# FitSNAP/FitSNAP

Measured on AMD Instinct MI355X. Metric: training rows/sec through A^T A + solve, 1000000 x 128 fp64 in total over the GPUs (strong scaling), higher is better.
Workload: dtype f64

## Files before the change

fitsnap_amd/build.py:

```python
from __future__ import annotations

import hashlib
import os
import shutil
import subprocess
import sys

HERE = os.path.dirname(os.path.abspath(__file__))
CSRC = os.path.join(HERE, "csrc")
LIBDIR = os.path.join(HERE, "_lib")
LIBNAME = "libfsnap_hip.so"
SOURCES = ["fsnap_syrk_quad.hip:0", "fsnap_syrk_quad.hip:1", "fsnap_syrk_quad.hip:2", "fsnap_syrk.hip", "fsnap_syrk_short.hip", "fsnap_rows.hip", "fsnap_chol.hip", "fsnap_trsm.hip", "fsnap_fused.hip", "fsnap_merr.hip", "fsnap_cand.hip", "fsnap_uq.hip", "fsnap_loco.hip", "fsnap_path.hip", "fsnap_joint.hip", "fsnap_select.hip", "fsnap_mcmc.hip", "fsnap_capi.cpp", "fsnap_comm.cpp", "fsnap_p2p.cpp",
           "fsnap_rowspace.cpp", "fsnap_rowspace_host.cpp", "fsnap_solve.cpp"]
HEADERS = ["fsnap_kernels.h", "fsnap_device_common.h", "fsnap_rowvar_body.h", "fsnap_ctx.h", "fsnap_rowspace_host.h", "fsnap_condest.h", "fsnap_p2p.h", os.path.join("..", "..", "include", "fsnap_hip.h")]
ARCH = "gfx950"


def lib_path() -> str:
    return os.path.join(LIBDIR, LIBNAME)


def _hipcc() -> str:
    exe = shutil.which("hipcc") or "/opt/rocm/bin/hipcc"
    if not os.path.exists(exe):
        raise RuntimeError("hipcc not found: libfsnap_hip.so cannot be built")
    return exe


def _source_digest() -> str:
    h = hashlib.sha256()
    for name in sorted({s.split(":")[0] for s in SOURCES}) + HEADERS:
        with open(os.path.join(CSRC, name), "rb") as f:
            h.update(f.read())
    return h.hexdigest()


def build_library(force: bool = False, verbose: bool = False) -> str:
    os.makedirs(LIBDIR, exist_ok=True)
    out = lib_path()
    stamp = out + ".sha256"
    digest = _source_digest()
    if not force and os.path.exists(out) and os.path.exists(stamp):
        with open(stamp) as f:
            if f.read().strip() == digest:
                return out
    hipcc = _hipcc()
    objs = []
    common = [f"--offload-arch={ARCH}", "-O3", "-std=c++17", "-fPIC", "-I", os.path.join(HERE, "..", "include")]
    procs = []
    objdir = os.path.join(LIBDIR, "obj")
    os.makedirs(objdir, exist_ok=True)
    hh = hashlib.sha256()
    for name in HEADERS:
        with open(os.path.join(CSRC, name), "rb") as f:
            hh.update(f.read())
    for entry in SOURCES:
        src, _, part = entry.partition(":")
        obj = os.path.join(objdir, os.path.splitext(src)[0] + (f"_{part}" if part else "") + ".o")
        cmd = [hipcc, *common]
        if part:
            cmd += [f"-DFSNAP_QUAD_PART={part}"]
        if src in ("fsnap_capi.cpp", "fsnap_comm.cpp", "fsnap_p2p.cpp", "fsnap_rowspace.cpp"):
            cmd += ["-x", "hip"]
        if src in ("fsnap_solve.cpp", "fsnap_rowspace_host.cpp"):
            cmd = [hipcc, "-x", "c++", "-O3", "-std=c++17", "-fPIC", "-mavx2", "-mfma",
# ... 39 lines not shown
```

fitsnap_amd/csrc/fsnap_capi.cpp:

```cpp
#include <hip/hip_runtime.h>

#include <algorithm>
#include <cmath>
#include <atomic>
#include <chrono>
#include <cstdarg>
#include <cstdio>
#include <cstdlib>
#include <cstring>
#include <limits>
#include <new>
#include <queue>
#include <string>
#include <thread>
#include <vector>

#include "../../include/fsnap_hip.h"
#include "fsnap_kernels.h"

extern "C" int fsnap_solve_diag_tagged(int kind, double param, int64_t K, const double* G, const double* c, const double* diag,
                                       double* beta, int* rank, double* rcond_est, int upper, const void* owner,
                                       unsigned long long generation);
extern "C" int fsnap_solve_diag_upper(int kind, double param, int64_t K, const double* G, const double* c, const double* diag,
                                      double* beta, int* rank, double* rcond_est);
// ... 526 lines not shown
    a.nblocks = g.nblocks;
    a.split = g.split;
    a.chunks_per_wave = g.cpw;
    a.nontemporal = true;
    a.part = (double*)ctx->part.p;
    a.cpart = (double*)ctx->cpart.p;
    a.spart = (double*)ctx->spart.p;
    int ns = -1;
    const double* spart_src = a.spart;
    if (g.fused_pack) {
        a.fused_pack = true;
    } else {
        int npk = 0;
        if ((rc = ensure_wpack(ctx, &npk))) return rc;
        a.wpack = ctx->wpack_override ? ctx->wpack_override : (const double*)ctx->wpack.p;
        spart_src = (const double*)ctx->wpack_spart.p;
        ns = npk;
    }
    hipEvent_t* evs;
    if ((rc = fit_events(ctx, &evs))) return rc;
    if (evs) FSNAP_HIP(hipEventRecord(evs[0], ctx->stream), "hipEventRecord");
    if (g.quad && g.cluster > 1) {
        const size_t need = (size_t)g.nblocks * 4 * sizeof(int);
        if (ctx->quad_flow.bytes < need) {
            if (!ctx->quad_flow.ensure(need)) return ctx->fail(FSNAP_E_NOMEM, "hipMalloc(flow words) failed");
            FSNAP_HIP(hipMemsetAsync(ctx->quad_flow.p, 0, ctx->quad_flow.bytes, ctx->stream), "hipMemset(flow words)");
            ctx->quad_flow_tag = 0;
        }
        ctx->quad_flow_tag += 1u << 20;
        a.flow_words = (int*)ctx->quad_flow.p;
        const int flow = 2 | ((g.cluster == 2 ? 0 : 2) << 2);
        a.flow_tag = (int)(ctx->quad_flow_tag | (unsigned)flow);
    }
    if (g.shortk) FSNAP_HIP(fsnap::launch_syrk_short(a, ctx->stream), "launch fsnap_syrk_short");
    else if (g.quad) FSNAP_HIP(fsnap::launch_syrk_quad(a, ctx->stream), "launch fsnap_syrk_quad");
    else if (g.acc) FSNAP_HIP(fsnap::launch_syrk_acc(a, ctx->stream), "launch fsnap_syrk_acc");
    else FSNAP_HIP(fsnap::launch_syrk_wave_p(a, ctx->stream), "launch fsnap_syrk_wave_p");
    if (evs) FSNAP_HIP(hipEventRecord(evs[1], ctx->stream), "hipEventRecord");
    double* mirror = nullptr;
    if (want_mirror && !device_factor(ctx, ctx->K)) {
        const size_t need = ((size_t)FSNAP_PACKED_LEN(ctx->K) + (size_t)ctx->K) * 8;
        if (ctx->mirror_bytes < need) {
            if (ctx->mirror) (void)hipHostFree(ctx->mirror);
            ctx->mirror = nullptr;
            ctx->mirror_bytes = 0;
            if (hipHostMalloc((void**)&ctx->mirror, need, hipHostMallocCoherent | hipHostMallocMapped) == hipSuccess)
                ctx->mirror_bytes = need;
        }
        if (ctx->mirror && !ctx->mirror_ev && hipEventCreateWithFlags(&ctx->mirror_ev, hipEventDisableTiming) != hipSuccess)
            ctx->mirror_ev = nullptr;
        if (ctx->mirror && ctx->mirror_ev) mirror = ctx->mirror;
    }
    const bool upper_mirror = mirror != nullptr;
    FSNAP_HIP(fsnap::launch_reduce(a.part, a.cpart, spart_src, g.nblocks, cs_per_block, ns, a.K, d_packed, mirror, accumulate,
                                   ctx->stream, upper_mirror),
              "launch fsnap_reduce_partials");
    if (evs) FSNAP_HIP(hipEventRecord(evs[2], ctx->stream), "hipEventRecord");
    if (mirror) {
        FSNAP_HIP(hipEventRecord(ctx->mirror_ev, ctx->stream), "hipEventRecord");
        ctx->mirror_of = d_packed;
        ctx->mirror_K = ctx->K;
        ctx->mirror_upper = upper_mirror;
        ctx->mirror_gen = next_mirror_generation();
    }
    if (evs) ctx->t_syrk = true;
    return FSNAP_OK;
}

}

namespace fsnap {

int wpack_current(fsnap_ctx* ctx) {
    int rc, npk = 0;
    if ((rc = check_rows(ctx)) || (rc = check_weights(ctx))) return rc;
    return ensure_wpack(ctx, &npk);
}

int normal_eq_launch_on(fsnap_ctx* ctx, const double* Q, int64_t ldq, const double* qpack, double* d_packed) {
    const double* const save_A = ctx->dA;
    const int64_t save_lda = ctx->lda;
    ctx->dA = Q;
    ctx->lda = ldq;
    ctx->wpack_override = qpack;
    const int rc = launch_normal_eq(ctx, d_packed);
    ctx->wpack_override = nullptr;
    ctx->dA = save_A;
    ctx->lda = save_lda;
    return rc;
}

}

extern "C" {

int fsnap_version(void) { return 200; }

int fsnap_device_count(int* count) {
    if (!count) return FSNAP_E_ARG;
    int n = 0;
    hipError_t e = hipGetDeviceCount(&n);
    if (e != hipSuccess) {
        g_last_error = std::string("hipGetDeviceCount: ") + hipGetErrorString(e);
        *count = 0;
        return FSNAP_E_HIP;
    }
    *count = n;
    return FSNAP_OK;
}
// ... 2180 lines not shown
```

fitsnap_amd/csrc/fsnap_kernels.h:

```cpp
#pragma once
#include <hip/hip_runtime.h>
#include <stdint.h>

namespace fsnap {

struct SyrkArgs {
    const double* A;
    int64_t lda;
    const double* b;
    const double* w;
    const unsigned char* mask;
    int64_t m;
    int K;
    int nblocks;
    int split;
    int64_t chunks_per_wave;
    bool nontemporal;
    double* part;
    double* cpart;
    double* spart;
    const double* wpack = nullptr;
    int* flow_words = nullptr;
    int flow_tag = 0;
    bool fused_pack = false;
};

struct TiledArgs {
    const double* A;
    int64_t lda;
    const double* wpack;
    int64_t m;
    int K;
    int NSB;
    int npairs;
    int nsplit;
    int64_t chunks_per_split;
    bool nontemporal;
    double* part;
    double* cpart;
    const double* spart;
    int ns;
};

int syrk_num_blocks(int K);
int syrk_waves_per_simd(int K, int split);
hipError_t launch_syrk_wave_p(const SyrkArgs& a, hipStream_t st);
hipError_t launch_syrk_acc(const SyrkArgs& a, hipStream_t st);
hipError_t launch_syrk_quad(const SyrkArgs& a, hipStream_t st);
int64_t syrk_quad_max_cpg();
int syrk_quad_cluster(int K);
int64_t syrk_acc_max_fused_cpw();
hipError_t launch_syrk_short(const SyrkArgs& a, hipStream_t st);
bool syrk_short_takes(int K);
int syrk_short_phase_rows(int K);
int64_t syrk_wave_p_max_fused_cpw(int K, int wg_per_cu);
hipError_t launch_reduce(const double* part, const double* cpart, const double* spart, int nblocks,
                         int cs_per_block, int ns, int K, double* out, double* mirror, bool accumulate, hipStream_t st,
                         bool upper_mirror = false);
int pack_weights_num_blocks(int64_t m);
hipError_t launch_pack_weights(const double* b, const double* w, const unsigned char* mask, int64_t m, double* wpack,
                               double* spart, hipStream_t st);
hipError_t launch_syrk_tiled(const TiledArgs& a, hipStream_t st);
hipError_t launch_reduce_tiled(const TiledArgs& a, double* out, bool accumulate, hipStream_t st);
hipError_t launch_weight_rows(const double* A, int64_t lda, const double* b, const double* w,
                              const unsigned char* mask, int64_t m, int K, double* aw, int64_t ldaw, double* bw,
                              hipStream_t st);
hipError_t launch_assemble(const double* raw, int64_t raw_ld, int64_t nrows, const int64_t* src_row, const int* kind,
                           const int* frac, const double* dval, const double* truth, const double* weight,
                           const double* fractions, const double* blank2J, int ntypes, int ncoeff, int off, double* A,
                           int64_t lda, double* b, double* w, hipStream_t st);
size_t assemble_row_record_bytes();
hipError_t launch_assemble_bw(const double* raw, int64_t raw_ld, int64_t nrows, const int64_t* src_row, const int* kind,
                              const int* frac, const double* d, const double* truth, const double* weight, int icolref,
                              double* b, double* w, void* recs, hipStream_t st);
hipError_t launch_assemble_syrk(const double* raw, int64_t raw_ld, const void* recs, const double* dval, const double* fractions,
                                const double* blank2J, int ntypes, int ncoeff, int off, const TiledArgs& a, hipStream_t st);
hipError_t launch_mirror_copy(const double* src, int K, double* mirror, hipStream_t st);
hipError_t launch_tri_pack(const double* packed, int K, double* tri, hipStream_t st);
hipError_t launch_tri_unpack(const double* tri, int K, double* packed, hipStream_t st);
size_t chol_large_work_doubles(int n);
hipError_t launch_chol_large(const double* packed, const double* cvec, int n, double alpha, double* work, double* dsc, double* z,
                             double* beta, int* status, double* minpiv, double* host_out, bool clear_status, double* probe_out,
                             hipStream_t st);
constexpr int CHOL_PROBES = 31;
double chol_probe(int row, int p);
hipError_t launch_chol_resolve(const double* d_rhs, int n, double* work, const double* dsc, double* z, double* beta, int* status,
                               const double* minpiv, double* host_out, hipStream_t st);
hipError_t launch_chol_factor(const double* G, int n, double shift, double* work, double* dsc, int* status, double* minpiv,
                              int K16, double* Rout, hipStream_t st);
hipError_t launch_gram_scan(const double* G, int n, double* out, hipStream_t st);
int gemv_num_blocks(int64_t m);
hipError_t launch_gemv_rows(const double* A, int64_t lda, const double* beta, int64_t m, int K, double* preds,
                            const double* b, const double* w, const unsigned char* mask, double* sse_part,
                            double* uout, hipStream_t st, bool uplain = false);
int gemvT_num_blocks(int64_t m);
int residual_num_blocks(int64_t m, int K);
hipError_t launch_residual_rows(const double* A, int64_t lda, const double* beta, int64_t m, int K, const double* b,
                                const double* w, const unsigned char* mask, double* partial, double* sse_part, double* out,
                                hipStream_t st);
hipError_t launch_colsum(const double* partial, int nparts, int ncols, double* out, hipStream_t st);
hipError_t launch_expand_weights(const double* wtrain, const unsigned char* mask, const int* rank, int64_t m, double* w,
                                 hipStream_t st);
int error_stats_num_blocks(int64_t m);
hipError_t launch_error_stats(const double* truth, const double* pred, const double* wgt, const int* cat, int64_t m, int ncat,
                              int pass, const double* means, double* partial, hipStream_t st);
hipError_t launch_gemvT_rows(const double* A, int64_t lda, const double* u, int64_t m, int K, double* partial,
                             double* out, hipStream_t st);

constexpr int MERR_IID = 0, MERR_ABC = 1, MERR_FULL = 2;
constexpr int MERR_ONE_PASS_MAX_K = 288;
int merr_num_blocks(int64_t m, int K);
// ... 97 lines not shown
```

fitsnap_amd/csrc/fsnap_solve.cpp:

```cpp
#include <atomic>
#include <chrono>
#include <cstdio>
#include <cmath>
#include <cstdlib>
#include <cstdint>
#include <cstring>
#include <limits>
#include <thread>
#include <vector>

#include "../../include/fsnap_hip.h"
#include "fsnap_condest.h"

static thread_local double g_cond_info[4] = {0.0, 0.0, 0.0, 0.0};

extern "C" __attribute__((visibility("hidden"))) void fsnap_cond_note(double min_pivot, double lambda_min, int steps, int where) {
    g_cond_info[0] = min_pivot;
    g_cond_info[1] = lambda_min;
    g_cond_info[2] = (double)steps;
    g_cond_info[3] = (double)where;
}

extern "C" int fsnap_cond_info(double* info) {
    if (!info) return FSNAP_E_ARG;
// ... 183 lines not shown
                *(v8du*)(r3) = y30; *(v8du*)(r3 + 8) = y31; *(v8du*)(r3 + 16) = y32; *(v8du*)(r3 + 24) = y33;
            }
        }
        if (cw == 16) {
            for (; i + 4 <= i_end; i += 4) {
                double* r0 = a + (size_t)i * n + c0;
                double* r1 = r0 + n;
                double* r2 = r1 + n;
                double* r3 = r2 + n;
                v8d y00 = *(const v8du*)(r0), y01 = *(const v8du*)(r0 + 8);
                v8d y10 = *(const v8du*)(r1), y11 = *(const v8du*)(r1 + 8);
                v8d y20 = *(const v8du*)(r2), y21 = *(const v8du*)(r2 + 8);
                v8d y30 = *(const v8du*)(r3), y31 = *(const v8du*)(r3 + 8);
                const double* uk = a + (size_t)jb * n;
                for (int k = 0; k < nk; ++k, uk += n) {
                    const v8d u0 = *(const v8du*)(uk + c0), u1 = *(const v8du*)(uk + c0 + 8);
                    const double f0 = uk[i], f1 = uk[i + 1], f2 = uk[i + 2], f3 = uk[i + 3];
                    const v8d b0 = {f0, f0, f0, f0, f0, f0, f0, f0}, b1 = {f1, f1, f1, f1, f1, f1, f1, f1};
                    const v8d b2 = {f2, f2, f2, f2, f2, f2, f2, f2}, b3 = {f3, f3, f3, f3, f3, f3, f3, f3};
                    y00 -= b0 * u0; y01 -= b0 * u1;
                    y10 -= b1 * u0; y11 -= b1 * u1;
                    y20 -= b2 * u0; y21 -= b2 * u1;
                    y30 -= b3 * u0; y31 -= b3 * u1;
                }
                *(v8du*)(r0) = y00; *(v8du*)(r0 + 8) = y01;
                *(v8du*)(r1) = y10; *(v8du*)(r1 + 8) = y11;
                *(v8du*)(r2) = y20; *(v8du*)(r2 + 8) = y21;
                *(v8du*)(r3) = y30; *(v8du*)(r3 + 8) = y31;
            }
        }
        for (; i < i_end; ++i) {
            double* ri = a + (size_t)i * n + c0;
            const double* uk = a + (size_t)jb * n;
            for (int k = 0; k < nk; ++k, uk += n) axpy_neg(ri, uk + c0, uk[i], cw);
        }
    }
}

int chol_upper_rb(double* a, int n, double* min_piv2, int NBK) {
    double mp = std::numeric_limits<double>::infinity();
    for (int jb = 0; jb < n; jb += NBK) {
        const int je = (jb + NBK < n) ? jb + NBK : n;
        const int fail = chol_panel(a, n, jb, je, &mp);
        if (fail >= 0) {
            if (min_piv2) *min_piv2 = mp;
            return fail;
        }
        if (je < n) chol_trailing_chunks(a, n, jb, je, 0, 1);
    }
    if (min_piv2) *min_piv2 = mp;
    return -1;
}

FSNAP_CLONES void chol_solve_inv(const double* u, int n, double* x, double* inv) {
    for (int k = 0; k < n; ++k) inv[k] = 1.0 / u[(size_t)k * n + k];
    for (int k = 0; k < n; ++k) {
        const double* r = u + (size_t)k * n;
        x[k] *= inv[k];
        axpy_neg(x + k + 1, r + k + 1, x[k], n - 1 - k);
    }
    for (int i = n - 1; i >= 0; --i) {
        const double* r = u + (size_t)i * n;
        x[i] = (x[i] - dotv(r + i + 1, x + i + 1, n - 1 - i)) * inv[i];
    }
}
void chol_solve(const double* u, int n, double* x) {
    static thread_local vec inv;
    inv.resize(n);
    chol_solve_inv(u, n, x, inv.data());
}

bool lu_solve(double* a, int n, double* b) {
    std::vector<int> piv(n);
    for (int j = 0; j < n; ++j) {
        int p = j;
        double mx = std::fabs(a[(size_t)j * n + j]);
        for (int i = j + 1; i < n; ++i) {
            double v = std::fabs(a[(size_t)i * n + j]);
            if (v > mx) {
                mx = v;
                p = i;
            }
        }
        if (!(mx > 0.0) || !std::isfinite(mx)) return false;
        if (p != j) {
            for (int k = 0; k < n; ++k) std::swap(a[(size_t)j * n + k], a[(size_t)p * n + k]);
            std::swap(b[j], b[p]);
        }
        const double inv = 1.0 / a[(size_t)j * n + j];
        for (int i = j + 1; i < n; ++i) {
            double f = a[(size_t)i * n + j] * inv;
            if (f == 0.0) continue;
            a[(size_t)i * n + j] = f;
            for (int k = j + 1; k < n; ++k) a[(size_t)i * n + k] -= f * a[(size_t)j * n + k];
            b[i] -= f * b[j];
        }
    }
    for (int i = n - 1; i >= 0; --i) {
        double s = b[i];
        for (int k = i + 1; k < n; ++k) s -= a[(size_t)i * n + k] * b[k];
        b[i] = s / a[(size_t)i * n + i];
    }
    return true;
}

void jacobi_eigh(double* a, int n, double* eval, double* v) {
    for (int i = 0; i < n; ++i)
        for (int j = 0; j < n; ++j) v[(size_t)i * n + j] = (i == j) ? 1.0 : 0.0;
    for (int sweep = 0; sweep < 60; ++sweep) {
        double off = 0.0, diag = 0.0;
        for (int i = 0; i < n; ++i) {
            diag += a[(size_t)i * n + i] * a[(size_t)i * n + i];
            for (int j = i + 1; j < n; ++j) off += a[(size_t)i * n + j] * a[(size_t)i * n + j];
        }
        if (off == 0.0 || off <= 1e-34 * diag) break;
        for (int p = 0; p < n - 1; ++p) {
            for (int q = p + 1; q < n; ++q) {
                const double apq = a[(size_t)p * n + q];
                if (apq == 0.0) continue;
                const double app = a[(size_t)p * n + p], aqq = a[(size_t)q * n + q];
                if (std::fabs(apq) <= 1e-18 * std::sqrt(std::fabs(app) * std::fabs(aqq))) {
                    a[(size_t)p * n + q] = a[(size_t)q * n + p] = 0.0;
// ... 172 lines not shown

int chol_upper_rb_mt(double* a, int n, double* min_piv2, int NBK, int nt) {
    struct Shared {
        std::atomic<int> arrived{0};
        std::atomic<int> phase{0};
        std::atomic<int> fail{-1};
        double mp = std::numeric_limits<double>::infinity();
    } sh;
    auto barrier = [&](int& local_phase) {
        ++local_phase;
        if (sh.arrived.fetch_add(1, std::memory_order_acq_rel) + 1 == nt) {
            sh.arrived.store(0, std::memory_order_relaxed);
            sh.phase.store(local_phase, std::memory_order_release);
        } else {
            int spins = 0;
            while (sh.phase.load(std::memory_order_acquire) != local_phase) {
#if defined(__x86_64__)
                __builtin_ia32_pause();
#endif
                if (++spins > 4096) {
                    std::this_thread::yield();
                    spins = 0;
                }
            }
        }
    };
    auto body = [&](int t) {
        int ph = 0;
        for (int jb = 0; jb < n; jb += NBK) {
            const int je = (jb + NBK < n) ? jb + NBK : n;
            if (t == 0) {
                const int f = chol_panel_diag(a, n, jb, je, &sh.mp);
                if (f >= 0) sh.fail.store(f, std::memory_order_relaxed);
            }
            barrier(ph);
            if (sh.fail.load(std::memory_order_relaxed) >= 0) return;
            if (je < n) {
                chol_panel_tails(a, n, jb, je, t, nt);
                barrier(ph);
                chol_trailing_chunks(a, n, jb, je, t, nt);
            }
            barrier(ph);
        }
    };
    std::vector<std::thread> th;
    th.reserve(nt - 1);
    for (int t = 1; t < nt; ++t) th.emplace_back(body, t);
    body(0);
    for (auto& x : th) x.join();
    if (min_piv2) *min_piv2 = sh.mp;
    return sh.fail.load();
}

int fast_chol(double* u, int n, double* mp2) {
    static const int forced = [] {
        const char* e = std::getenv("FSNAP_CHOL_VARIANT");
        return e ? std::atoi(e) : 0;
    }();
    static const int nbk_env = [] {
        const char* e = std::getenv("FSNAP_CHOL_NBK");
        return e ? std::atoi(e) : 0;
    }();
    if (forced == 1) return chol_upper(u, n, mp2);
    if (forced == 2) return chol_upper_blocked(u, n, mp2, 64);
    if (forced == 3 || n >= 48) {
        const int nbk = nbk_env > 0 ? nbk_env : (n <= 256 ? 8 : 32);
        static const int nt_env = [] {
            const char* e = std::getenv("FSNAP_CHOL_THREADS");
            return e ? std::atoi(e) : 0;
        }();
        static const int nt_auto = [] {
            auto quota = [](const char* path, bool v2) -> bool {
                FILE* f = std::fopen(path, "r");
                if (!f) return false;
                char buf[64] = {0};
                const bool got = std::fgets(buf, sizeof buf, f) != nullptr;
                std::fclose(f);
                if (!got) return false;
                return v2 ? std::strncmp(buf, "max", 3) != 0 : std::atol(buf) > 0;
            };
            if (quota("/sys/fs/cgroup/cpu.max", true) || quota("/sys/fs/cgroup/cpu/cpu.cfs_quota_us", false)) return 1;
            const unsigned hc = std::thread::hardware_concurrency();
            return (int)(hc >= 8 ? 8 : (hc > 0 ? hc : 1));
        }();
        int nt = nt_env > 0 ? nt_env : nt_auto;
        if (nt > n / 160) nt = n / 160;
        if (nt > 1) return chol_upper_rb_mt(u, n, mp2, nbk, nt);
        return chol_upper_rb(u, n, mp2, nbk);
    }
    return chol_upper(u, n, mp2);
}

}

namespace {
struct PhaseTimer {
    bool on;
    std::chrono::steady_clock::time_point t0;
    PhaseTimer() : on(std::getenv("FSNAP_SOLVE_TIMING") != nullptr), t0(std::chrono::steady_clock::now()) {}
    void lap(const char* what) {
        if (!on) return;
        const auto t1 = std::chrono::steady_clock::now();
        std::fprintf(stderr, "[fsnap_solve] %-14s %9.1f us\n", what, std::chrono::duration<double, std::micro>(t1 - t0).count());
        t0 = t1;
    }
};
}

extern "C" int fsnap_solve_diag(int kind, double param, int64_t K64, const double* G, const double* c, const double* diag,
                                double* beta, int* rank_out, double* rcond_est);
extern "C" int fsnap_solve_diag_upper(int kind, double param, int64_t K64, const double* G, const double* c, const double* diag,
                                      double* beta, int* rank_out, double* rcond_est);
namespace {
int solve_impl(int kind, double param, int64_t K64, const double* G, const double* c, const double* diag, double* beta,
               int* rank_out, double* rcond_est, bool upper_only, const void* owner = nullptr, unsigned long long generation = 0);
}

extern "C" __attribute__((visibility("hidden"))) int fsnap_host_chol_upper(double* a, int n, double* min_piv) {
    return fast_chol(a, n, min_piv);
}

extern "C" __attribute__((visibility("hidden"))) double fsnap_gen_eig_max(const double* M, const double* N, int k) {
    if (k <= 0 || !all_finite(M, (size_t)k * k) || !all_finite(N, (size_t)k * k)) return -1.0;
    vec U(N, N + (size_t)k * k), C((size_t)k * k);
    for (int i = 0; i < k; ++i)
        for (int j = 0; j < i; ++j) U[(size_t)i * k + j] = 0.0;
    double mp = 0.0;
    if (chol_upper(U.data(), k, &mp) >= 0) return -1.0;
    vec T(M, M + (size_t)k * k);
    auto forward_columns = [&](vec& X) {
        for (int i = 0; i < k; ++i) {
            const double inv = 1.0 / U[(size_t)i * k + i];
            for (int c = 0; c < k; ++c) {
                double sacc = X[(size_t)i * k + c];
                for (int l = 0; l < i; ++l) sacc -= U[(size_t)l * k + i] * X[(size_t)l * k + c];
                X[(size_t)i * k + c] = sacc * inv;
            }
        }
    };
    forward_columns(T);
    for (int i = 0; i < k; ++i)
        for (int j = 0; j < k; ++j) C[(size_t)i * k + j] = T[(size_t)j * k + i];
    forward_columns(C);
    for (int i = 0; i < k; ++i)
        for (int j = i + 1; j < k; ++j) C[(size_t)i * k + j] = C[(size_t)j * k + i] = 0.5 * (C[(size_t)i * k + j] + C[(size_t)j * k + i]);
    const double* Cp = C.data();
    vec tmp((size_t)k);
    const fsnap::CondEstimate top = fsnap::lanczos_lambda_min(k, [Cp, k, &tmp](double* x) {
        for (int i = 0; i < k; ++i) {
            double acc = 0.0;
            for (int j = 0; j < k; ++j) acc += Cp[(size_t)i * k + j] * x[j];
            tmp[i] = acc;
        }
        for (int i = 0; i < k; ++i) x[i] = tmp[i];
        return true;
    }, 4, 16);
    return top.lambda_min > 0.0 && std::isfinite(top.lambda_min) ? 1.0 / top.lambda_min : -1.0;
}

extern "C" int fsnap_solve(int kind, double param, int64_t K64, const double* G, const double* c, double* beta,
                           int* rank_out, double* rcond_est) {
    return fsnap_solve_diag(kind, param, K64, G, c, nullptr, beta, rank_out, rcond_est);
}

extern "C" __attribute__((visibility("hidden"))) int fsnap_solve_diag(int kind, double param, int64_t K64, const double* G,
                                                                      const double* c, const double* diag, double* beta,
                                                                      int* rank_out, double* rcond_est) {
    return solve_impl(kind, param, K64, G, c, diag, beta, rank_out, rcond_est, false);
}

extern "C" __attribute__((visibility("hidden"))) int fsnap_solve_diag_upper(int kind, double param, int64_t K64, const double* G,
                                                                            const double* c, const double* diag, double* beta,
                                                                            int* rank_out, double* rcond_est) {
    return solve_impl(kind, param, K64, G, c, diag, beta, rank_out, rcond_est, true);
}

extern "C" __attribute__((visibility("hidden"))) int fsnap_solve_diag_tagged(int kind, double param, int64_t K64, const double* G,
                                                                             const double* c, const double* diag, double* beta,
                                                                             int* rank_out, double* rcond_est, int upper,
                                                                             const void* owner, unsigned long long generation) {
    return solve_impl(kind, param, K64, G, c, diag, beta, rank_out, rcond_est, upper != 0, owner, generation);
}

namespace {
int solve_impl(int kind, double param, int64_t K64, const double* G, const double* c, const double* diag, double* beta,
               int* rank_out, double* rcond_est, bool upper_only, const void* owner, unsigned long long generation) {
    PhaseTimer timer;
    if (!G || !c || !beta || K64 <= 0 || K64 > (1 << 20)) return FSNAP_E_ARG;
    if (kind < FSNAP_SOLVE_CHOL || kind > FSNAP_SOLVE_RIDGE_INV_PROBE) return FSNAP_E_ARG;
    const bool probe = kind >= FSNAP_SOLVE_LSTSQ_PROBE;
    if (kind == FSNAP_SOLVE_LSTSQ_PROBE) kind = FSNAP_SOLVE_LSTSQ;
    if (kind == FSNAP_SOLVE_RIDGE_PROBE) kind = FSNAP_SOLVE_RIDGE;
    if (kind == FSNAP_SOLVE_RIDGE_INV_PROBE) kind = FSNAP_SOLVE_RIDGE_INV;
    const int K = (int)K64;
    if (!std::isfinite(param)) return FSNAP_NUM_NONFINITE;
    const double alpha = (kind == FSNAP_SOLVE_RIDGE || kind == FSNAP_SOLVE_RIDGE_INV) ? param : 0.0;
    const double eps = std::numeric_limits<double>::epsilon();
    timer.lap("finite check");

    {
        int Kp = (K >= 48 && (K & 15) != 0) ? ((K + 15) & ~15) : K;
        if (Kp >= 384 && (Kp & 127) == 0) Kp += 32;
        static thread_local vec U, dsc, z;
        static thread_local struct { const void* owner; unsigned long long gen; int K; double alpha, mp2, piv, lam; } held = {nullptr, 0, 0, 0.0, 0.0, 0.0, 0.0};
        if (owner && held.owner == owner && held.gen == generation && held.K == K && held.alpha == alpha &&
            U.size() == (size_t)Kp * Kp) {
            bool fin = true;
            for (int i = 0; i < K; ++i) {
                z[i] = c[i] * dsc[i];
                fin = fin && (c[i] - c[i] == 0.0);
            }
            if (fin) {
                for (int i = K; i < Kp; ++i) z[i] = 0.0;
                chol_solve(U.data(), Kp, z.data());
                for (int i = 0; i < K; ++i) beta[i] = z[i] * dsc[i];
                timer.lap("tri solves (factor reused)");
                if (all_finite(beta, K)) {
                    if (rank_out) *rank_out = K;
                    if (rcond_est) *rcond_est = held.mp2;
                    fsnap_cond_note(held.piv, held.lam, 0, 0);
                    return FSNAP_OK;
                }
            }
        }
        held.owner = nullptr;
        U.resize((size_t)Kp * Kp);
        dsc.resize(Kp);
        z.resize(Kp);
        bool ok = true;
        double chk = 0.0;
        for (int i = 0; i < K && ok; ++i) {
            const double g = (diag ? diag[i] : G[(size_t)i * K + i]) + alpha;
            if (!(g > 0.0) || !std::isfinite(g)) ok = false;
            else dsc[i] = 1.0 / std::sqrt(g);
            chk += c[i] * 0.0;
        }
        timer.lap("diag scale");
        if (ok) {
            const v8d zero = {0, 0, 0, 0, 0, 0, 0, 0};
            v8d chk0 = zero, chk1 = zero;
            for (int i = 0; i < K; ++i) {
                const double* gi = G + (size_t)i * K;
                double* ui = U.data() + (size_t)i * Kp;
                const double di = dsc[i];
                const v8d dv = {di, di, di, di, di, di, di, di};
                const int j0 = i & ~7;
                if (i + 2 < K) {
                    const double* gn = G + (size_t)(i + 2) * K;
                    for (int jp = (i + 2) & ~7; jp < K; jp += 8) __builtin_prefetch(gn + jp, 0, 0);
                }
                int j = 0;
                for (; j + 8 <= j0; j += 8) *(v8du*)(ui + j) = zero;
                if (upper_only && j + 8 <= K) {
                    typedef long long v8l __attribute__((vector_size(64)));
                    const v8l lanes = {0, 1, 2, 3, 4, 5, 6, 7};
                    const v8l keep = (lanes + (long long)j) >= (long long)i;
                    const v8d g0 = (v8d)((v8l)(*(const v8du*)(gi + j)) & keep);
                    chk0 += g0 * zero;
                    *(v8du*)(ui + j) = g0 * dv * *(const v8du*)(dsc.data() + j);
                    j += 8;
                }
                for (; j + 16 <= K; j += 16) {
                    const v8d g0 = *(const v8du*)(gi + j), g1 = *(const v8du*)(gi + j + 8);
                    chk0 += g0 * zero;
                    chk1 += g1 * zero;
                    *(v8du*)(ui + j) = g0 * dv * *(const v8du*)(dsc.data() + j);
                    *(v8du*)(ui + j + 8) = g1 * dv * *(const v8du*)(dsc.data() + j + 8);
                }
                for (; j + 8 <= K; j += 8) {
                    const v8d g0 = *(const v8du*)(gi + j);
                    chk0 += g0 * zero;
                    *(v8du*)(ui + j) = g0 * dv * *(const v8du*)(dsc.data() + j);
                }
                for (; j < K; ++j) {
                    const double gij = (upper_only && j < i) ? 0.0 : gi[j];
                    ui[j] = gij * di * dsc[j];
                    chk += gij * 0.0;
                }
                for (; j < Kp; ++j) ui[j] = 0.0;
                ui[i] = (gi[i] + alpha) * di * di;
            }
            for (int i = K; i < Kp; ++i) {
                double* ui = U.data() + (size_t)i * Kp;
                for (int j = 0; j < Kp; ++j) ui[j] = 0.0;
                ui[i] = 1.0;
            }
            const v8d cs = chk0 + chk1;
            chk += ((cs[0] + cs[1]) + (cs[2] + cs[3])) + ((cs[4] + cs[5]) + (cs[6] + cs[7]));
            double mp2 = 0.0;
            timer.lap("scale/build");
            const bool fact_ok = (chk == 0.0) && fast_chol(U.data(), Kp, &mp2) < 0;
            timer.lap("cholesky");
            fsnap::CondEstimate ce;
            bool cond_ok = true;
            if (fact_ok && mp2 > 1.0e-3 && kind == FSNAP_SOLVE_LSTSQ) {
                const double* Up = U.data();
                ce = fsnap::lanczos_lambda_min(Kp, [Up, Kp](double* v) {
                    chol_solve(Up, Kp, v);
                    return true;
                });
                cond_ok = ce.lambda_min > 64.0 * K * eps;
                timer.lap("cond estimate");
            }
            if (fact_ok && mp2 > 1.0e-3 && cond_ok) {
                const double piv = mp2;
                if (ce.steps && ce.lambda_min < mp2) mp2 = ce.lambda_min;
                fsnap_cond_note(piv, ce.lambda_min, ce.steps, 0);
                for (int i = 0; i < K; ++i) z[i] = c[i] * dsc[i];
                for (int i = K; i < Kp; ++i) z[i] = 0.0;
                chol_solve(U.data(), Kp, z.data());
                for (int i = 0; i < K; ++i) beta[i] = z[i] * dsc[i];
                timer.lap("tri solves");
                if (all_finite(beta, K)) {
                    if (rank_out) *rank_out = K;
                    if (rcond_est) *rcond_est = mp2;
                    if (owner) {
                        held.owner = owner;
                        held.gen = generation;
                        held.K = K;
                        held.alpha = alpha;
                        held.mp2 = mp2;
                        held.piv = piv;
                        held.lam = ce.lambda_min;
                    }
                    return FSNAP_OK;
                }
            }
        }
    }

    static thread_local vec Gfull;
    if (upper_only) {
        Gfull.resize((size_t)K * K);
        for (int i = 0; i < K; ++i)
            for (int j = i; j < K; ++j) Gfull[(size_t)i * K + j] = Gfull[(size_t)j * K + i] = G[(size_t)i * K + j];
        G = Gfull.data();
    }
    if (!all_finite(G, (size_t)K * K) || !all_finite(c, K)) return FSNAP_NUM_NONFINITE;
    static thread_local Reduced R;
    R.idx.clear();
    R.idx.reserve(K);
    for (int j = 0; j < K; ++j) {
        const double gjj = G[(size_t)j * K + j] + alpha;
        if (gjj == 0.0 && kind != FSNAP_SOLVE_CHOL && kind != FSNAP_SOLVE_RIDGE_INV) continue;
        R.idx.push_back(j);
    }
    const int n = R.n = (int)R.idx.size();
    for (int j = 0; j < K; ++j) beta[j] = 0.0;
    if (rank_out) *rank_out = 0;
    if (rcond_est) *rcond_est = 0.0;
    if (n == 0) return FSNAP_OK;
    R.M.resize((size_t)n * n);
    R.rhs.resize(n);
    for (int i = 0; i < n; ++i) {
        R.rhs[i] = c[R.idx[i]];
        for (int j = 0; j < n; ++j) {
            const double gij = 0.5 * (G[(size_t)R.idx[i] * K + R.idx[j]] + G[(size_t)R.idx[j] * K + R.idx[i]]);
            R.M[(size_t)i * n + j] = gij + ((i == j) ? alpha : 0.0);
        }
    }

    vec x;
    double mp2 = 0.0;
// ... 112 lines not shown
```

Measured before the change: 3.097 billion.

## Add fused partial-reduce finish kernel and small-K augmented Cholesky solve

Adds a new fsnap_finish kernel that reduces the SYRK partials with a 16-slice shared-memory reduction. It is used whenever a host mirror is requested or the block count is small; otherwise the old reduce kernel still runs. On the host, for padded K between 48 and 144 it switches to a panelled 4-row Cholesky. The right-hand side is appended as an extra column so the forward solve is fused into the factorisation, leaving only a backward substitution. It also deepens prefetching and skips zeroing the lower triangle. The aim is to cut reduce-kernel and host-solve latency for K=128, at the cost of more specialised code paths to keep correct.

```diff
diff --git a/fitsnap_amd/build.py b/fitsnap_amd/build.py
--- a/fitsnap_amd/build.py
+++ b/fitsnap_amd/build.py
@@ -10,7 +10,7 @@
 CSRC = os.path.join(HERE, "csrc")
 LIBDIR = os.path.join(HERE, "_lib")
 LIBNAME = "libfsnap_hip.so"
-SOURCES = ["fsnap_syrk_quad.hip:0", "fsnap_syrk_quad.hip:1", "fsnap_syrk_quad.hip:2", "fsnap_syrk.hip", "fsnap_syrk_short.hip", "fsnap_rows.hip", "fsnap_chol.hip", "fsnap_trsm.hip", "fsnap_fused.hip", "fsnap_merr.hip", "fsnap_cand.hip", "fsnap_uq.hip", "fsnap_loco.hip", "fsnap_path.hip", "fsnap_joint.hip", "fsnap_select.hip", "fsnap_mcmc.hip", "fsnap_capi.cpp", "fsnap_comm.cpp", "fsnap_p2p.cpp",
+SOURCES = ["fsnap_syrk_quad.hip:0", "fsnap_syrk_quad.hip:1", "fsnap_syrk_quad.hip:2", "fsnap_syrk.hip", "fsnap_syrk_short.hip", "fsnap_finish.hip", "fsnap_rows.hip", "fsnap_chol.hip", "fsnap_trsm.hip", "fsnap_fused.hip", "fsnap_merr.hip", "fsnap_cand.hip", "fsnap_uq.hip", "fsnap_loco.hip", "fsnap_path.hip", "fsnap_joint.hip", "fsnap_select.hip", "fsnap_mcmc.hip", "fsnap_capi.cpp", "fsnap_comm.cpp", "fsnap_p2p.cpp",
            "fsnap_rowspace.cpp", "fsnap_rowspace_host.cpp", "fsnap_solve.cpp"]
 HEADERS = ["fsnap_kernels.h", "fsnap_device_common.h", "fsnap_rowvar_body.h", "fsnap_ctx.h", "fsnap_rowspace_host.h", "fsnap_condest.h", "fsnap_p2p.h", os.path.join("..", "..", "include", "fsnap_hip.h")]
 ARCH = "gfx950"
diff --git a/fitsnap_amd/csrc/fsnap_capi.cpp b/fitsnap_amd/csrc/fsnap_capi.cpp
--- a/fitsnap_amd/csrc/fsnap_capi.cpp
+++ b/fitsnap_amd/csrc/fsnap_capi.cpp
@@ -602,9 +602,14 @@
         if (ctx->mirror && ctx->mirror_ev) mirror = ctx->mirror;
     }
     const bool upper_mirror = mirror != nullptr;
-    FSNAP_HIP(fsnap::launch_reduce(a.part, a.cpart, spart_src, g.nblocks, cs_per_block, ns, a.K, d_packed, mirror, accumulate,
-                                   ctx->stream, upper_mirror),
-              "launch fsnap_reduce_partials");
+    if (mirror || g.NB <= 9)
+        FSNAP_HIP(fsnap::launch_finish(a.part, a.cpart, spart_src, g.nblocks, cs_per_block, ns, a.K, d_packed, mirror, accumulate,
+                                       ctx->stream, upper_mirror),
+                  "launch fsnap_finish");
+    else
+        FSNAP_HIP(fsnap::launch_reduce(a.part, a.cpart, spart_src, g.nblocks, cs_per_block, ns, a.K, d_packed, mirror, accumulate,
+                                       ctx->stream, upper_mirror),
+                  "launch fsnap_reduce_partials");
     if (evs) FSNAP_HIP(hipEventRecord(evs[2], ctx->stream), "hipEventRecord");
     if (mirror) {
         FSNAP_HIP(hipEventRecord(ctx->mirror_ev, ctx->stream), "hipEventRecord");
diff --git a/fitsnap_amd/csrc/fsnap_finish.hip b/fitsnap_amd/csrc/fsnap_finish.hip
--- /dev/null
+++ b/fitsnap_amd/csrc/fsnap_finish.hip
@@ -0,0 +1,135 @@
+#include "fsnap_device_common.h"
+#include "fsnap_kernels.h"
+
+namespace {
+
+__host__ __device__ constexpr int fin_tri_index(int p, int q, int NB) { return p * NB - (p * (p - 1)) / 2 + (q - p); }
+
+__device__ inline int fin_col_of(int bq, int e, int NB) {
+    if ((NB & 1) && bq == NB - 1) return 16 * bq + e;
+    return 32 * (bq >> 1) + 2 * e + (bq & 1);
+}
+
+__global__ __launch_bounds__(256) void fsnap_finish_k(const double* __restrict__ part, const double* __restrict__ cpart,
+                                                      const double* __restrict__ spart, int nblocks, int cs_per_block, int ns,
+                                                      int NB, int K, double* __restrict__ out, double* __restrict__ mirror,
+                                                      int accumulate, int upper_mirror) {
+    __shared__ __attribute__((aligned(16))) double red[16][32];
+    const int NTILE = NB * (NB + 1) / 2;
+    const int nG = NTILE * 256, nC = NB * 16;
+    const int gG = nG / 32, gC = (nC + 31) / 32;
+    const int tid = threadIdx.x, sub = tid & 15, slice = tid >> 4;
+    const int b = blockIdx.x;
+    int region, e0, nel, np;
+    const double* src;
+    int64_t stride;
+    int tp = 0, tq = 0, piece = 0;
+    bool paired = false;
+    if (b < gG) {
+        region = 0; e0 = b * 32; nel = nG; np = nblocks; src = part; stride = nG;
+        const int t = b >> 3;
+        while (tp + 1 < NB && fin_tri_index(tp + 1, tp + 1, NB) <= t) ++tp;
+        tq = tp + (t - fin_tri_index(tp, tp, NB));
+        paired = (tq | 1) < (NB & ~1) && (tq & ~1) >= tp;
+        piece = (b & 7) + 8 * (tq & 1);
+    } else if (b < gG + gC) {
+        region = 1; e0 = (b - gG) * 32; nel = nC; np = nblocks * cs_per_block; src = cpart; stride = nC;
+    } else {
+        region = 2; e0 = 0; nel = 4; np = ns >= 0 ? ns : nblocks * cs_per_block; src = spart; stride = 4;
+    }
+    int el = e0 + 2 * sub;
+    if (paired) {
+        const int tile = fin_tri_index(tp, tq & ~1, NB) + (sub >> 3);
+        el = tile * 256 + piece * 16 + 2 * (sub & 7);
+    }
+    d2 a0 = {0.0, 0.0}, a1 = a0, a2 = a0, a3 = a0;
+    if (el < nel) {
+        const double* s0 = src + el;
+        int p = slice;
+        for (; p + 240 < np; p += 256) {
+            d2 x[16];
+#pragma unroll
+            for (int j = 0; j < 16; ++j) x[j] = *reinterpret_cast<const d2*>(s0 + (int64_t)(p + 16 * j) * stride);
+#pragma unroll
+            for (int j = 0; j < 16; j += 4) {
+                a0 += x[j];
+                a1 += x[j + 1];
+                a2 += x[j + 2];
+                a3 += x[j + 3];
+            }
+        }
+        for (; p < np; p += 16) a0 += *reinterpret_cast<const d2*>(s0 + (int64_t)p * stride);
+    }
+    const d2 sv = (a0 + a1) + (a2 + a3);
+    if (paired) {
+        const int c0 = 4 * (sub & 7) + (sub >> 3);
+        red[slice][c0] = sv.x;
+        red[slice][c0 + 2] = sv.y;
+    } else {
+        *reinterpret_cast<d2*>(&red[slice][2 * sub]) = sv;
+    }
+    __syncthreads();
+    if (tid >= 32) return;
+    const int idx = e0 + tid;
+    if (!paired && idx >= nel) return;
+    double tot = red[0][tid];
+#pragma unroll
+    for (int k = 1; k < 16; ++k) tot += red[k][tid];
+    if (region == 0) {
+        int q, ep, eq;
+        if (paired) {
+            q = (tq & ~1) + (tid & 1);
+            ep = piece;
+            eq = tid >> 1;
+        } else {
+            const int rem = idx & 255, i = rem >> 6, ln = rem & 63;
+            q = tq;
+            ep = (ln >> 4) + 4 * i;
+            eq = ln & 15;
+        }
+        const int p = tp;
+        const int r = fin_col_of(p, ep, NB), c = fin_col_of(q, eq, NB);
+        if (r < K && c < K) {
+            const double val = accumulate ? out[(int64_t)r * K + c] + tot : tot;
+            out[(int64_t)r * K + c] = val;
+            if (p != q) out[(int64_t)c * K + r] = val;
+            if (mirror) {
+                if (upper_mirror) {
+                    const int lo = r < c ? r : c, hi = r < c ? c : r;
+                    if (p != q) mirror[(int64_t)lo * K + hi] = val;
+                    else mirror[(int64_t)r * K + c] = val;
+                } else {
+                    mirror[(int64_t)r * K + c] = val;
+                    if (p != q) mirror[(int64_t)c * K + r] = val;
+                }
+                if (r == c) mirror[(int64_t)K * K + K + 3 + r] = val;
+            }
+        }
+    } else if (region == 1) {
+        const int cidx = fin_col_of(idx >> 4, idx & 15, NB);
+        if (cidx < K) {
+            const double val = accumulate ? out[(int64_t)K * K + cidx] + tot : tot;
+            out[(int64_t)K * K + cidx] = val;
+            if (mirror) mirror[(int64_t)K * K + cidx] = val;
+        }
+    } else if (idx < 3) {
+        const double val = accumulate ? out[(int64_t)K * K + K + idx] + tot : tot;
+        out[(int64_t)K * K + K + idx] = val;
+        if (mirror) mirror[(int64_t)K * K + K + idx] = val;
+    }
+}
+
+}
+
+namespace fsnap {
+
+hipError_t launch_finish(const double* part, const double* cpart, const double* spart, int nblocks, int cs_per_block, int ns,
+                         int K, double* out, double* mirror, bool accumulate, hipStream_t st, bool upper_mirror) {
+    const int NB = syrk_num_blocks(K);
+    const int ngroups = NB * (NB + 1) / 2 * 8 + (NB * 16 + 31) / 32 + 1;
+    hipLaunchKernelGGL(fsnap_finish_k, dim3((unsigned)ngroups), dim3(256), 0, st, part, cpart, spart, nblocks, cs_per_block, ns,
+                       NB, K, out, mirror, accumulate ? 1 : 0, upper_mirror ? 1 : 0);
+    return hipGetLastError();
+}
+
+}
diff --git a/fitsnap_amd/csrc/fsnap_kernels.h b/fitsnap_amd/csrc/fsnap_kernels.h
--- a/fitsnap_amd/csrc/fsnap_kernels.h
+++ b/fitsnap_amd/csrc/fsnap_kernels.h
@@ -57,6 +57,8 @@
 hipError_t launch_reduce(const double* part, const double* cpart, const double* spart, int nblocks,
                          int cs_per_block, int ns, int K, double* out, double* mirror, bool accumulate, hipStream_t st,
                          bool upper_mirror = false);
+hipError_t launch_finish(const double* part, const double* cpart, const double* spart, int nblocks, int cs_per_block, int ns,
+                         int K, double* out, double* mirror, bool accumulate, hipStream_t st, bool upper_mirror = false);
 int pack_weights_num_blocks(int64_t m);
 hipError_t launch_pack_weights(const double* b, const double* w, const unsigned char* mask, int64_t m, double* wpack,
                                double* spart, hipStream_t st);
diff --git a/fitsnap_amd/csrc/fsnap_solve.cpp b/fitsnap_amd/csrc/fsnap_solve.cpp
--- a/fitsnap_amd/csrc/fsnap_solve.cpp
+++ b/fitsnap_amd/csrc/fsnap_solve.cpp
@@ -259,22 +259,164 @@
     return -1;
 }
 
-FSNAP_CLONES void chol_solve_inv(const double* u, int n, double* x, double* inv) {
-    for (int k = 0; k < n; ++k) inv[k] = 1.0 / u[(size_t)k * n + k];
+FSNAP_CLONES void chol_solve_inv(const double* u, int n, int ld, double* x, double* inv) {
+    for (int k = 0; k < n; ++k) inv[k] = 1.0 / u[(size_t)k * ld + k];
     for (int k = 0; k < n; ++k) {
-        const double* r = u + (size_t)k * n;
+        const double* r = u + (size_t)k * ld;
         x[k] *= inv[k];
         axpy_neg(x + k + 1, r + k + 1, x[k], n - 1 - k);
     }
     for (int i = n - 1; i >= 0; --i) {
-        const double* r = u + (size_t)i * n;
+        const double* r = u + (size_t)i * ld;
         x[i] = (x[i] - dotv(r + i + 1, x + i + 1, n - 1 - i)) * inv[i];
     }
 }
-void chol_solve(const double* u, int n, double* x) {
+void chol_solve(const double* u, int n, double* x, int ld = 0) {
     static thread_local vec inv;
     inv.resize(n);
-    chol_solve_inv(u, n, x, inv.data());
+    chol_solve_inv(u, n, ld > 0 ? ld : n, x, inv.data());
+}
+FSNAP_CLONES void chol_backward(const double* u, int n, int ld, double* x, const double* inv) {
+    for (int i = n - 1; i >= 0; --i) {
+        const double* r = u + (size_t)i * ld;
+        x[i] = (x[i] - dotv(r + i + 1, x + i + 1, n - 1 - i)) * inv[i];
+    }
+}
+
+template <int NV, bool DIAG>
+FSNAP_INLINE int chol_small_group(double* a, int ld, int i, int c, double* invd, double* mp) {
+    double* r0 = a + (size_t)i * ld + c;
+    double* r1 = r0 + ld;
+    double* r2 = r1 + ld;
+    double* r3 = r2 + ld;
+    v8d y0[NV], y1[NV], y2[NV], y3[NV];
+#pragma unroll
+    for (int v = 0; v < NV; ++v) {
+        y0[v] = *(const v8du*)(r0 + 8 * v);
+        y1[v] = *(const v8du*)(r1 + 8 * v);
+        y2[v] = *(const v8du*)(r2 + 8 * v);
+        y3[v] = *(const v8du*)(r3 + 8 * v);
+    }
+    const double* uk = a + c;
+    const double* fk = a + i;
+    for (int k = 0; k < i; ++k, uk += ld, fk += ld) {
+        const double f0 = fk[0], f1 = fk[1], f2 = fk[2], f3 = fk[3];
+        const v8d b0 = {f0, f0, f0, f0, f0, f0, f0, f0}, b1 = {f1, f1, f1, f1, f1, f1, f1, f1};
+        const v8d b2 = {f2, f2, f2, f2, f2, f2, f2, f2}, b3 = {f3, f3, f3, f3, f3, f3, f3, f3};
+#pragma unroll
+        for (int v = 0; v < NV; ++v) {
+            const v8d u = *(const v8du*)(uk + 8 * v);
+            y0[v] -= b0 * u;
+            y1[v] -= b1 * u;
+            y2[v] -= b2 * u;
+            y3[v] -= b3 * u;
+        }
+    }
+    if (!DIAG) {
+        const double* g = a + (size_t)i * ld + i;
+        const double s0 = invd[i], s1 = invd[i + 1], s2 = invd[i + 2], s3 = invd[i + 3];
+        const double f01 = g[1], f02 = g[2], f03 = g[3], f12 = g[ld + 2], f13 = g[ld + 3], f23 = g[2 * ld + 3];
+        const v8d w0 = {s0, s0, s0, s0, s0, s0, s0, s0}, w1 = {s1, s1, s1, s1, s1, s1, s1, s1};
+        const v8d w2 = {s2, s2, s2, s2, s2, s2, s2, s2}, w3 = {s3, s3, s3, s3, s3, s3, s3, s3};
+        const v8d e01 = {f01, f01, f01, f01, f01, f01, f01, f01}, e02 = {f02, f02, f02, f02, f02, f02, f02, f02};
+        const v8d e03 = {f03, f03, f03, f03, f03, f03, f03, f03}, e12 = {f12, f12, f12, f12, f12, f12, f12, f12};
+        const v8d e13 = {f13, f13, f13, f13, f13, f13, f13, f13}, e23 = {f23, f23, f23, f23, f23, f23, f23, f23};
+#pragma unroll
+        for (int v = 0; v < NV; ++v) {
+            v8d t0 = y0[v], t1 = y1[v], t2 = y2[v], t3 = y3[v];
+            t0 *= w0;
+            t1 -= e01 * t0;
+            t2 -= e02 * t0;
+            t3 -= e03 * t0;
+            t1 *= w1;
+            t2 -= e12 * t1;
+            t3 -= e13 * t1;
+            t2 *= w2;
+            t3 -= e23 * t2;
+            t3 *= w3;
+            *(v8du*)(r0 + 8 * v) = t0;
+            *(v8du*)(r1 + 8 * v) = t1;
+            *(v8du*)(r2 + 8 * v) = t2;
+            *(v8du*)(r3 + 8 * v) = t3;
+        }
+        return -1;
+    }
+#pragma unroll
+    for (int v = 0; v < NV; ++v) {
+        *(v8du*)(r0 + 8 * v) = y0[v];
+        *(v8du*)(r1 + 8 * v) = y1[v];
+        *(v8du*)(r2 + 8 * v) = y2[v];
+        *(v8du*)(r3 + 8 * v) = y3[v];
+    }
+    for (int r = 0; r < 4; ++r) {
+        double* rr = r0 + (size_t)r * ld;
+        const int dl = i + r - c;
+        const double d = rr[dl];
+        if (d < *mp) *mp = d;
+        if (!(d > 0.0) || !std::isfinite(d)) return i + r;
+        const double rt = std::sqrt(d), inv = 1.0 / rt;
+        invd[i + r] = inv;
+        const v8d iv = {inv, inv, inv, inv, inv, inv, inv, inv}, rtv = {rt, rt, rt, rt, rt, rt, rt, rt};
+        typedef long long v8l __attribute__((vector_size(64)));
+        const v8l lanes = {0, 1, 2, 3, 4, 5, 6, 7};
+#pragma unroll
+        for (int v = 0; v < NV; ++v) {
+            v8d t = *(const v8du*)(rr + 8 * v);
+            t *= iv;
+            const v8l at = (lanes + (long long)(8 * v)) == (long long)dl;
+            *(v8du*)(rr + 8 * v) = (v8d)(((v8l)t & ~at) | ((v8l)rtv & at));
+        }
+        for (int q = r + 1; q < 4; ++q) {
+            double* rq = r0 + (size_t)q * ld;
+            const double f = rr[dl + (q - r)];
+            const v8d fv = {f, f, f, f, f, f, f, f};
+#pragma unroll
+            for (int v = 0; v < NV; ++v) {
+                v8d t = *(const v8du*)(rq + 8 * v);
+                t -= fv * *(const v8du*)(rr + 8 * v);
+                *(v8du*)(rq + 8 * v) = t;
+            }
+        }
+    }
+    return -1;
+}
+
+template <bool DIAG>
+FSNAP_INLINE int chol_small_dispatch(int nv, double* a, int ld, int i, int c, double* invd, double* mp) {
+    switch (nv) {
+        case 1: return chol_small_group<1, DIAG>(a, ld, i, c, invd, mp);
+        case 2: return chol_small_group<2, DIAG>(a, ld, i, c, invd, mp);
+        case 3: return chol_small_group<3, DIAG>(a, ld, i, c, invd, mp);
+        case 4: return chol_small_group<4, DIAG>(a, ld, i, c, invd, mp);
+        default: return chol_small_group<5, DIAG>(a, ld, i, c, invd, mp);
+    }
+}
+
+FSNAP_CLONES int chol_small(double* a, int n, int ld, double* invd, double* min_piv2) {
+    double mp = std::numeric_limits<double>::infinity();
+    const int V = ld >> 3, npanel = (V + 4) / 5;
+    int v0 = 0;
+    for (int pn = 0; pn < npanel; ++pn) {
+        const int v1 = v0 + (V - v0) / (npanel - pn);
+        const int c0 = 8 * v0, c1 = 8 * v1;
+        const int i_end = c1 < n ? c1 : n;
+        int fail = -1;
+        for (int i = 0; i < i_end && fail < 0; i += 4) {
+            if (i + 4 <= c0) {
+                fail = chol_small_dispatch<false>(v1 - v0, a, ld, i, c0, invd, &mp);
+            } else {
+                const int cs = i & ~7;
+                fail = chol_small_dispatch<true>((c1 - cs) >> 3, a, ld, i, cs, invd, &mp);
+            }
+        }
+        if (fail >= 0) {
+            *min_piv2 = mp;
+            return fail;
+        }
+        v0 = v1;
+    }
+    *min_piv2 = mp;
+    return -1;
 }
 
 bool lu_solve(double* a, int n, double* b) {
@@ -553,15 +695,22 @@
     return sh.fail.load();
 }
 
+int chol_env(const char* name) {
+    const char* e = std::getenv(name);
+    return e ? std::atoi(e) : 0;
+}
+int chol_forced_variant() {
+    static const int forced = chol_env("FSNAP_CHOL_VARIANT");
+    return forced;
+}
+int chol_forced_nbk() {
+    static const int nbk = chol_env("FSNAP_CHOL_NBK");
+    return nbk;
+}
+
 int fast_chol(double* u, int n, double* mp2) {
-    static const int forced = [] {
-        const char* e = std::getenv("FSNAP_CHOL_VARIANT");
-        return e ? std::atoi(e) : 0;
-    }();
-    static const int nbk_env = [] {
-        const char* e = std::getenv("FSNAP_CHOL_NBK");
-        return e ? std::atoi(e) : 0;
-    }();
+    const int forced = chol_forced_variant();
+    const int nbk_env = chol_forced_nbk();
     if (forced == 1) return chol_upper(u, n, mp2);
     if (forced == 2) return chol_upper_blocked(u, n, mp2, 64);
     if (forced == 3 || n >= 48) {
@@ -598,7 +747,13 @@
 struct PhaseTimer {
     bool on;
     std::chrono::steady_clock::time_point t0;
-    PhaseTimer() : on(std::getenv("FSNAP_SOLVE_TIMING") != nullptr), t0(std::chrono::steady_clock::now()) {}
+    static bool enabled() {
+        static const bool e = std::getenv("FSNAP_SOLVE_TIMING") != nullptr;
+        return e;
+    }
+    PhaseTimer() : on(enabled()) {
+        if (on) t0 = std::chrono::steady_clock::now();
+    }
     void lap(const char* what) {
         if (!on) return;
         const auto t1 = std::chrono::steady_clock::now();
@@ -702,10 +857,13 @@
     {
         int Kp = (K >= 48 && (K & 15) != 0) ? ((K + 15) & ~15) : K;
         if (Kp >= 384 && (Kp & 127) == 0) Kp += 32;
-        static thread_local vec U, dsc, z;
+        const bool small = Kp >= 48 && Kp <= 144 && chol_forced_variant() == 0 && chol_forced_nbk() == 0;
+        const int ld = small ? Kp + 8 : Kp;
+        static thread_local vec U, dsc, z, invd;
+        constexpr int SMALL_PF_ROWS = 4;
         static thread_local struct { const void* owner; unsigned long long gen; int K; double alpha, mp2, piv, lam; } held = {nullptr, 0, 0, 0.0, 0.0, 0.0, 0.0};
         if (owner && held.owner == owner && held.gen == generation && held.K == K && held.alpha == alpha &&
-            U.size() == (size_t)Kp * Kp) {
+            U.size() == (size_t)Kp * ld) {
             bool fin = true;
             for (int i = 0; i < K; ++i) {
                 z[i] = c[i] * dsc[i];
@@ -713,7 +871,7 @@
             }
             if (fin) {
                 for (int i = K; i < Kp; ++i) z[i] = 0.0;
-                chol_solve(U.data(), Kp, z.data());
+                chol_solve(U.data(), Kp, z.data(), ld);
                 for (int i = 0; i < K; ++i) beta[i] = z[i] * dsc[i];
                 timer.lap("tri solves (factor reused)");
                 if (all_finite(beta, K)) {
@@ -725,9 +883,19 @@
             }
         }
         held.owner = nullptr;
-        U.resize((size_t)Kp * Kp);
+        U.resize((size_t)Kp * ld);
         dsc.resize(Kp);
         z.resize(Kp);
+        if (small) {
+            invd.resize(Kp);
+            for (int j = 0; j < K; j += 8) __builtin_prefetch(c + j, 0, 3);
+            if (diag)
+                for (int j = 0; j < K; j += 8) __builtin_prefetch(diag + j, 0, 3);
+            for (int i = 0; i < SMALL_PF_ROWS && i < K; ++i) {
+                const double* gi = G + (size_t)i * K;
+                for (int j = i & ~7; j < K; j += 8) __builtin_prefetch(gi + j, 0, 0);
+            }
+        }
         bool ok = true;
         double chk = 0.0;
         for (int i = 0; i < K && ok; ++i) {
@@ -738,25 +906,31 @@
         }
         timer.lap("diag scale");
         if (ok) {
+            double mp2 = 0.0;
+            bool fact_ok;
+            const int pf = small ? SMALL_PF_ROWS : 2;
             const v8d zero = {0, 0, 0, 0, 0, 0, 0, 0};
             v8d chk0 = zero, chk1 = zero;
             for (int i = 0; i < K; ++i) {
                 const double* gi = G + (size_t)i * K;
-                double* ui = U.data() + (size_t)i * Kp;
+                double* ui = U.data() + (size_t)i * ld;
                 const double di = dsc[i];
                 const v8d dv = {di, di, di, di, di, di, di, di};
-                const int j0 = i & ~7;
-                if (i + 2 < K) {
-                    const double* gn = G + (size_t)(i + 2) * K;
-                    for (int jp = (i + 2) & ~7; jp < K; jp += 8) __builtin_prefetch(gn + jp, 0, 0);
-                }
-                int j = 0;
-                for (; j + 8 <= j0; j += 8) *(v8du*)(ui + j) = zero;
-                if (upper_only && j + 8 <= K) {
-                    typedef long long v8l __attribute__((vector_size(64)));
-                    const v8l lanes = {0, 1, 2, 3, 4, 5, 6, 7};
-                    const v8l keep = (lanes + (long long)j) >= (long long)i;
-                    const v8d g0 = (v8d)((v8l)(*(const v8du*)(gi + j)) & keep);
+                if (i + pf < K) {
+                    const double* gn = G + (size_t)(i + pf) * K;
+                    for (int jp = (i + pf) & ~7; jp < K; jp += 8) __builtin_prefetch(gn + jp, 0, 0);
+                }
+                int j = i & ~7;
+                if (!small)
+                    for (int jz = 0; jz < j; jz += 8) *(v8du*)(ui + jz) = zero;
+                if (j + 8 <= K) {
+                    v8d g0 = *(const v8du*)(gi + j);
+                    if (upper_only) {
+                        typedef long long v8l __attribute__((vector_size(64)));
+                        const v8l lanes = {0, 1, 2, 3, 4, 5, 6, 7};
+                        const v8l keep = (lanes + (long long)j) >= (long long)i;
+                        g0 = (v8d)((v8l)g0 & keep);
+                    }
                     chk0 += g0 * zero;
                     *(v8du*)(ui + j) = g0 * dv * *(const v8du*)(dsc.data() + j);
                     j += 8;
@@ -778,26 +952,31 @@
                     ui[j] = gij * di * dsc[j];
                     chk += gij * 0.0;
                 }
-                for (; j < Kp; ++j) ui[j] = 0.0;
+                for (; j < ld; ++j) ui[j] = 0.0;
+                if (small) ui[Kp] = c[i] * di;
                 ui[i] = (gi[i] + alpha) * di * di;
             }
             for (int i = K; i < Kp; ++i) {
-                double* ui = U.data() + (size_t)i * Kp;
-                for (int j = 0; j < Kp; ++j) ui[j] = 0.0;
+                double* ui = U.data() + (size_t)i * ld;
+                for (int j = small ? (i & ~7) : 0; j < ld; ++j) ui[j] = 0.0;
                 ui[i] = 1.0;
             }
             const v8d cs = chk0 + chk1;
             chk += ((cs[0] + cs[1]) + (cs[2] + cs[3])) + ((cs[4] + cs[5]) + (cs[6] + cs[7]));
-            double mp2 = 0.0;
             timer.lap("scale/build");
-            const bool fact_ok = (chk == 0.0) && fast_chol(U.data(), Kp, &mp2) < 0;
-            timer.lap("cholesky");
+            if (small) {
+                fact_ok = (chk == 0.0) && chol_small(U.data(), Kp, ld, invd.data(), &mp2) < 0;
+                timer.lap("cholesky+fwd");
+            } else {
+                fact_ok = (chk == 0.0) && fast_chol(U.data(), Kp, &mp2) < 0;
+                timer.lap("cholesky");
+            }
             fsnap::CondEstimate ce;
             bool cond_ok = true;
             if (fact_ok && mp2 > 1.0e-3 && kind == FSNAP_SOLVE_LSTSQ) {
                 const double* Up = U.data();
-                ce = fsnap::lanczos_lambda_min(Kp, [Up, Kp](double* v) {
-                    chol_solve(Up, Kp, v);
+                ce = fsnap::lanczos_lambda_min(Kp, [Up, Kp, ld](double* v) {
+                    chol_solve(Up, Kp, v, ld);
                     return true;
                 });
                 cond_ok = ce.lambda_min > 64.0 * K * eps;
@@ -807,9 +986,14 @@
                 const double piv = mp2;
                 if (ce.steps && ce.lambda_min < mp2) mp2 = ce.lambda_min;
                 fsnap_cond_note(piv, ce.lambda_min, ce.steps, 0);
-                for (int i = 0; i < K; ++i) z[i] = c[i] * dsc[i];
-                for (int i = K; i < Kp; ++i) z[i] = 0.0;
-                chol_solve(U.data(), Kp, z.data());
+                if (small) {
+                    for (int i = 0; i < Kp; ++i) z[i] = U[(size_t)i * ld + Kp];
+                    chol_backward(U.data(), Kp, ld, z.data(), invd.data());
+                } else {
+                    for (int i = 0; i < K; ++i) z[i] = c[i] * dsc[i];
+                    for (int i = K; i < Kp; ++i) z[i] = 0.0;
+                    chol_solve(U.data(), Kp, z.data());
+                }
                 for (int i = 0; i < K; ++i) beta[i] = z[i] * dsc[i];
                 timer.lap("tri solves");
                 if (all_finite(beta, K)) {
```

After: 3.068 billion. Within noise of the previous version (-0.9%).
